# michelerenzullo/Blur_algorithms

Hardware: AMD Instinct MI355X
Metric: megapixels/sec Gaussian blur (σ=20, 4K RGB) at 1/2/4/8 GPUs; % HBM roofline (higher is better)
Workload: dtype f16 hi+lo operands (u8 pixels exact, taps and intermediate split in two binary16 halves), f32 accumulate

## Files before the change

### blur_algorithms_amd/csrc/fw_kernels.hpp

```cpp
#pragma once
#include "fx_kernels.hpp"
#include <type_traits>

#ifndef FW_TL_REGS
#define FW_TL_REGS 12
#endif

namespace blur_amd {

typedef uint32_t FwChSel;
constexpr FwChSel fw_chsel_all(int ch) { return static_cast<FwChSel>(ch) | (ch > 1 ? 0xe40u : 0u); }
inline FwChSel fw_chsel_mask(unsigned mask, int ch)
{
    FwChSel s = 0;
    int n = 0;
    for (int c = 0; c < ch; ++c)
        if (mask >> c & 1u) s |= static_cast<FwChSel>(c) << (4 + 2 * n++);
    return s | static_cast<FwChSel>(n);
}
__host__ __device__ constexpr int fw_chsel_count(FwChSel s) { return static_cast<int>(s & 7u); }
inline unsigned fw_chsel_bits(FwChSel s)
{
    unsigned m = 0;
    for (int i = 0; i < fw_chsel_count(s); ++i) m |= 1u << ((s >> (4 + 2 * i)) & 3u);
// ... 256 lines not shown
            } else {
#pragma unroll
                for (int k = 8 * hf; k < 8 * hf + 8; ++k) sv[k] = arow[k] * kFxRowUnscale;
            }
        } else if (sub == 1 || sub == 2) {
#pragma unroll
            for (int k = 4 * hf + 2 * (sub - 1); k < 4 * hf + 2 * sub; ++k) {
                typedef float f2 __attribute__((ext_vector_type(2)));
                typedef _Float16 h2 __attribute__((ext_vector_type(2)));
                const f2 vv = { sv[2 * k], sv[2 * k + 1] };
                hp[k] = __builtin_bit_cast(uint32_t, __builtin_convertvector(vv, h2));
                float r0, r1;
                mx_remainder(hp[k], vv[0], vv[1], r0, r1);
                const f2 rem = { r0, r1 };
                lp[k] = __builtin_bit_cast(uint32_t, __builtin_convertvector(rem, h2));
            }
        } else {
            fx_swap4(hp[4 * hf], hp[4 * hf + 2], hp[4 * hf + 1], hp[4 * hf + 3], lp[4 * hf], lp[4 * hf + 2], lp[4 * hf + 1], lp[4 * hf + 3]);
        }
    };
    const uint32_t sel1 = (lane & 1) ? 0x03070105u : 0x06020400u, sel2 = (lane & 2) ? 0x03020706u : 0x05040100u;
    auto emit_piece = [&](int gq) __attribute__((always_inline)) {
        float fv[4];
#pragma unroll
        for (int k = 0; k < 4; ++k) {
            const int reg = 4 * gq + k;
            fv[k] = __builtin_fmaf(tfin[reg], kMxUnscale, (reg & 1) ? cneg : cpos);
        }
        const uint32_t b0 = static_cast<uint32_t>(static_cast<int>(fv[0])) & 0xffu, b1 = static_cast<uint32_t>(static_cast<int>(fv[1])) & 0xffu;
        const uint32_t b2 = static_cast<uint32_t>(static_cast<int>(fv[2])) & 0xffu, b3 = static_cast<uint32_t>(static_cast<int>(fv[3]));
        const uint32_t pk = b0 | (b1 << 8) | (b2 << 16) | (b3 << 24);
        rr[gq] = CH == 1 ? fx_quad_transpose(pk, sel1, sel2) : pk;
    };
    auto colpass = [&](int qs, int hb, int ri, auto beside) __attribute__((always_inline)) {
        mx_half8 v1[2], v2[2];
#pragma unroll
        for (int b = 0; b < 2; ++b) {
            const u4 w1 = { hl[hb][0][4 * b], hl[hb][0][4 * b + 1], hl[hb][0][4 * b + 2], hl[hb][0][4 * b + 3] };
            const u4 w2 = { hl[hb][1][4 * b], hl[hb][1][4 * b + 1], hl[hb][1][4 * b + 2], hl[hb][1][4 * b + 3] };
            v1[b] = __builtin_bit_cast(mx_half8, w1);
            v2[b] = __builtin_bit_cast(mx_half8, w2);
        }
        auto dof = [](int it) { return it == 0 ? NKB - 1 : (it >= NKB - 2 ? it - (NKB - 2) : it + 1); };
        mx_half8 tq[3];
        tq[0] = tlo(dof(0));
        if (NKB > 1) tq[1] = tlo(dof(1));
#pragma unroll
        for (int it = 0; it < CS; ++it) {
            if (it < NKB) {
                const int d = dof(it);
                const int b = d & 1, a2 = d >> 1, slot = (qs - a2 + 2 * NT) % NT;
                if (it + 2 < NKB) tq[(it + 2) % 3] = tlo(dof(it + 2));
                if (ri < 0 || a2 <= ri) {
                    mx_float16 t = d == 0 ? zero : acc[slot];
                    t = __builtin_amdgcn_mfma_f32_32x32x16_f16(th[d], v1[b], t, 0, 0, 0);
                    t = __builtin_amdgcn_mfma_f32_32x32x16_f16(tq[it % 3], v1[b], t, 0, 0, 0);
                    t = __builtin_amdgcn_mfma_f32_32x32x16_f16(th[d], v2[b], t, 0, 0, 0);
                    asm volatile("" : "+a"(t));
                    if (it == 0) tfin = t; else acc[slot] = t;
                }
            }
            beside(it);
            __builtin_amdgcn_sched_barrier(0);
        }
    };
    const __amdgpu_buffer_rsrc_t rout = __builtin_amdgcn_make_buffer_rsrc(out, 0, static_cast<uint32_t>(g.rows - 1) * pt.dst_pitch + static_cast<uint32_t>(g.cols) * CH, kMxRsrcWord3);
    const int xcol = x0 + 32 * wave + m;
    const uint32_t lane_out = CH == 3 ? static_cast<uint32_t>(4 * h) * pt.dst_pitch + static_cast<uint32_t>(xcol) * CH + static_cast<uint32_t>(c) : 0u;
    uint32_t rowstep_ = pt.dst_pitch;
    asm volatile("" : "+s"(rowstep_));
    const uint32_t rowstep = rowstep_;
    const int xq = x0 + 32 * wave + 4 * (m >> 2), q = m & 3;
    const bool ragged = (g.cols & 3) != 0;
    const int qn = xq >= g.cols ? 0 : min(4, g.cols - xq);
    auto store_group = [&](int tile, bool valid, int gq) __attribute__((always_inline)) {
        const uint32_t v = rr[gq];
        if constexpr (CH == 1) {
            const int row = 32 * tile + 8 * gq + 4 * h + q;
            const bool rok = valid && row < g.rows;
            const uint32_t o = static_cast<uint32_t>(row) * rowstep + static_cast<uint32_t>(xq);
            __builtin_amdgcn_raw_buffer_store_b32(v, rout, rok && qn == 4 ? o : 0xfffffff0u, 0, 0);
            if (ragged) {
#pragma unroll
                for (int k = 0; k < 3; ++k)
                    __builtin_amdgcn_raw_buffer_store_b8(static_cast<uint8_t>(v >> (8 * k)), rout, rok && qn < 4 && k < qn ? o + k : 0xfffffff0u, 0, 0);
            }
        } else {
            int row0 = 32 * tile + 8 * gq + 4 * h;
            if constexpr (CH == 4) asm volatile("" : "+v"(row0));
            const uint32_t base = CH == 3 ? lane_out + static_cast<uint32_t>(32 * tile + 8 * gq) * rowstep
                                          : static_cast<uint32_t>(row0) * rowstep + static_cast<uint32_t>(xcol) * CH + static_cast<uint32_t>(c);
#pragma unroll
            for (int k = 0; k < 4; ++k) {
                const bool ok = valid && xcol < g.cols && row0 + k < g.rows;
                __builtin_amdgcn_raw_buffer_store_b8(static_cast<uint8_t>(v >> (8 * k)), rout, ok ? base + k * rowstep : 0xfffffff0u, 0, 0);
            }
        }
    };

    issue_window(s0);
#pragma unroll
    for (int k = 0; k < PER; ++k) commit_item(0, k);
    commit_q(0);
    issue_window(s0 + 1);
#pragma unroll
    for (int k = 0; k < PER; ++k) commit_item(1, k);
    commit_q(1);
    __syncthreads();
    rowpass(0, [](int) {});
#pragma unroll
    for (int p = 0; p < 8; ++p) split_piece(0, 0, p);
    __syncthreads();

    auto step = [&](int s, int qs, int ri) __attribute__((always_inline)) {
        const int par = (s - s0) & 1;
        const int ptile = s - 1 - NT;
        const bool pvalid = ptile >= tile0 && s > s0;
        issue_window(s + 2);
        rowpass(par ^ 1, [&](int kb) __attribute__((always_inline)) {
            if (kb < 4) store_group(ptile, pvalid, kb);
        });
        colpass(qs, 0, ri, [&](int it) __attribute__((always_inline)) {
            if (it < 8) split_piece(par ^ 1, 1, it);
            if (it >= 1 && it <= 4) emit_piece(it - 1);
            if (it >= 5) {
#pragma unroll
                for (int i = 0; i < IPS; ++i) commit_item(par, IPS * (it - 5) + i);
            }
            if (it == CS - 1) commit_q(par);
        });
#pragma unroll
        for (int k = 0; k < 8; ++k) { hl[0][0][k] = hl[1][0][k]; hl[0][1][k] = hl[1][1][k]; }
        __syncthreads();
    };
#pragma unroll
    for (int j = 0; j < NT; ++j) step(s0 + j, j, j);
    for (int sb = s0 + NT; sb < s1; sb += NT) {
#pragma unroll
        for (int qs = 0; qs < NT; ++qs) {
            const int s = sb + qs;
            if (s >= s1) break;
            step(s, qs, -1);
        }
    }
    {
        const int ltile = s1 - 1 - NT;
#pragma unroll
        for (int gq = 0; gq < 4; ++gq) store_group(ltile, ltile >= tile0, gq);
    }
}

template <int NKB, int CH> hipError_t fw_launch(hipStream_t st, const uint8_t* src, uint8_t* dst, const void* frags, FxGeom g, int num_cus, const FwQuirk<CH>* qk,
                                               const uint8_t* strips, FwChSel chsel, FwPitch pt)
{
    using C = FwCfg<NKB>;
    const int nact = fw_chsel_count(chsel);
    if (nact < 1 || nact > CH) return hipErrorInvalidValue;
    for (int i = 0; i < nact; ++i)
        if (static_cast<int>((chsel >> (4 + 2 * i)) & 3u) >= CH) return hipErrorInvalidValue;
    const FxLaunch l = fx_plan_launch(g, nact, C::NT, num_cus);
    if (l.ntasks == 0) return hipSuccess;
    static std::atomic<unsigned long long> attr_done{ 0 };
    const hipError_t e = fx_set_lds(attr_done, C::LDS, fw_blur_u8<NKB, true, CH>, fw_blur_u8<NKB, false, CH>);
    if (e != hipSuccess) return e;
    if (qk)
        hipLaunchKernelGGL((fw_blur_u8<NKB, true, CH>), l.grid, dim3(256), C::LDS, st, src, dst, static_cast<const mx_half8*>(frags), g, l.chunks, l.tps,
                           l.nseg, static_cast<int>(l.ntasks), *qk, strips, chsel, pt);
    else
        hipLaunchKernelGGL((fw_blur_u8<NKB, false, CH>), l.grid, dim3(256), C::LDS, st, src, dst, static_cast<const mx_half8*>(frags), g, l.chunks, l.tps,
                           l.nseg, static_cast<int>(l.ntasks), FwQuirk<CH>{}, strips, chsel, pt);
    return hipGetLastError();
}

template <int NKB> hipError_t fw_launch_u8c3(hipStream_t st, const uint8_t* src, uint8_t* dst, const void* frags, FxGeom g, int num_cus, const FxQuirk* qk,
                                             const uint8_t* strips, float* vdump, unsigned long long* stamps)
{
// ... 170 lines not shown
```

### blur_algorithms_amd/csrc/fx_kernels.hpp

```cpp
#pragma once
#include "mx_kernels.hpp"
#include <atomic>

#if !defined(FX_NO_SGB) && !defined(FX_SGB)
#define FX_SGB 1
#endif
#ifndef FX_SGB_A
#define FX_SGB_A 5
#endif
#ifndef FX_SGB_B
#define FX_SGB_B 6
#endif

namespace blur_amd {

struct FxGeom {
    int rows, cols, pad;
    int nframes;
    int aligned;
    int ntiles;
    int nright;
    int nxcd;
};

// ... 23 lines not shown
constexpr float kFxRowUnscale = 1024.f;

__host__ __device__ constexpr uint32_t fx_sel1(int B, int da, int db) { return (B >> 2) == db ? static_cast<uint32_t>(B & 3) : static_cast<uint32_t>(4 + (B & 3)); }

template <int NKB> struct FxRaw { uint32_t d[FxCfg<NKB>::PER][3]; };

__device__ __forceinline__ void fx_swap4(uint32_t& a0, uint32_t& b0, uint32_t& a1, uint32_t& b1, uint32_t& a2, uint32_t& b2, uint32_t& a3, uint32_t& b3)
{
    asm("s_nop 1\n\tv_permlane32_swap_b32 %0, %1\n\tv_permlane32_swap_b32 %2, %3\n\tv_permlane32_swap_b32 %4, %5\n\tv_permlane32_swap_b32 %6, %7"
        : "+v"(a0), "+v"(b0), "+v"(a1), "+v"(b1), "+v"(a2), "+v"(b2), "+v"(a3), "+v"(b3));
}

template <int CTRL> __device__ __forceinline__ uint32_t fx_dpp(uint32_t x)
{
    return static_cast<uint32_t>(__builtin_amdgcn_update_dpp(0, static_cast<int>(x), CTRL, 0xf, 0xf, true));
}

#ifdef FX_ABL_M16
typedef float fx_f4 __attribute__((ext_vector_type(4)));
struct fx_tile { fx_f4 q[4]; };
#define FX_EL(t, i) ((t).q[(i) >> 2][(i) & 3])
#define FX_PIN(t) asm volatile("" : "+a"((t).q[0]), "+a"((t).q[1]), "+a"((t).q[2]), "+a"((t).q[3]))
__device__ __forceinline__ void fx_mma(mx_half8 a, mx_half8 b, fx_tile& t, int pair)
{
    t.q[2 * pair] = __builtin_amdgcn_mfma_f32_16x16x32_f16(a, b, t.q[2 * pair], 0, 0, 0);
    t.q[2 * pair + 1] = __builtin_amdgcn_mfma_f32_16x16x32_f16(a, b, t.q[2 * pair + 1], 0, 0, 0);
}
#else
typedef mx_float16 fx_tile;
#define FX_EL(t, i) ((t)[i])
#define FX_PIN(t) asm volatile("" : "+a"(t))
__device__ __forceinline__ void fx_mma(mx_half8 a, mx_half8 b, fx_tile& t, int) { t = __builtin_amdgcn_mfma_f32_32x32x16_f16(a, b, t, 0, 0, 0); }
#endif

__device__ __forceinline__ uint32_t fx_quad_transpose(uint32_t p, uint32_t sel1, uint32_t sel2)
{
    const uint32_t t = fx_dpp<0xb1>(p);
    const uint32_t q = __builtin_amdgcn_perm(t, p, sel1);
    const uint32_t u = fx_dpp<0x4e>(q);
    return __builtin_amdgcn_perm(u, q, sel2);
}

struct FxQuirk {
    const int* srow_part;
    const int* cpart;
    const long long* zpart;
    const float* taps;
    int nbatches, nbands;
    int cpitch;
    float dr, dc;
};

template <int NCH>
__device__ __forceinline__ void fx_quirk_cols_tile(unsigned char* scratch, float* qc, const FxQuirk& q, int f, int x0, int c0, int cols, int pad, int tid)
{
    const int win = kFxChunk + 2 * pad, nval = NCH * win, ntap = 2 * pad + 1;
    double* cc = reinterpret_cast<double*>(scratch);
    double* tp = cc + nval;
    double* zs = tp + ntap;
    int* S = reinterpret_cast<int*>(zs + 4 + ((nval + ntap) & 1));
    const size_t bstride = static_cast<size_t>(q.cpitch);
    const int wlo = x0 - pad, whi = min(x0 + kFxChunk, cols) + pad;
    int xlo = max(wlo, 0), xhi = min(whi, cols);
    if (wlo < 0) xhi = max(xhi, min(cols, 1 - wlo));
    if (whi > cols) xlo = min(xlo, max(0, 2 * cols - 1 - whi));
    {
// ... 236 lines not shown
    };
    float sv[16];
    auto split_piece = [&](int buf, int c, int piece, int sprod = 0) __attribute__((always_inline)) {
        const int hf = piece / 4, sub = piece % 4;
        uint32_t (&hp)[8] = hl[0];
        uint32_t (&lp)[8] = hl[1];
#ifdef FX_ABL_NOSPLIT
        if (sub == 0) {
#pragma unroll
            for (int k = 0; k < 4; ++k) { hp[4 * hf + k] = __builtin_bit_cast(uint32_t, FX_EL(arow, 8 * hf + k)); lp[4 * hf + k] = __builtin_bit_cast(uint32_t, FX_EL(arow, 8 * hf + 4 + k)); }
        }
        return;
#endif
        if (sub == 0) {
            if (QUIRK) {
                const float* qs4 = reinterpret_cast<const float*>(fx_lds + C::QOFF) + buf * 512 + (m & 1) * 256 + c * 32 + 4 * h;
#pragma unroll
                for (int k = 0; k < 2; ++k) {
                    const float4 t4 = *reinterpret_cast<const float4*>(qs4 + 8 * (2 * hf + k));
                    sv[8 * hf + 4 * k] = __builtin_fmaf(FX_EL(arow, 8 * hf + 4 * k), kFxRowUnscale, t4.x);
                    sv[8 * hf + 4 * k + 1] = __builtin_fmaf(FX_EL(arow, 8 * hf + 4 * k + 1), kFxRowUnscale, t4.y);
                    sv[8 * hf + 4 * k + 2] = __builtin_fmaf(FX_EL(arow, 8 * hf + 4 * k + 2), kFxRowUnscale, t4.z);
                    sv[8 * hf + 4 * k + 3] = __builtin_fmaf(FX_EL(arow, 8 * hf + 4 * k + 3), kFxRowUnscale, t4.w);
                }
            } else {
#pragma unroll
                for (int k = 0; k < 8; ++k) sv[8 * hf + k] = FX_EL(arow, 8 * hf + k) * kFxRowUnscale;
            }
            if (DUMPV) {
                const int x = x0 + 32 * wave + m;
#pragma unroll
                for (int k = 0; k < 8; ++k) {
                    const int reg = 8 * hf + k, r = 32 * sprod + (reg & 3) + 8 * (reg >> 2) + 4 * h - PADA;
                    if (r >= 0 && r < g.rows && x < g.cols) vdump[((static_cast<size_t>(f) * 3 + c) * g.rows + r) * g.cols + x] = sv[8 * hf + k];
                }
            }
        } else if (sub == 1 || sub == 2) {
#pragma unroll
            for (int k = 2 * (sub - 1); k < 2 * sub; ++k) {
                typedef float f2 __attribute__((ext_vector_type(2)));
                typedef _Float16 h2 __attribute__((ext_vector_type(2)));
                const f2 vv = { sv[8 * hf + 2 * k], sv[8 * hf + 2 * k + 1] };
                hp[4 * hf + k] = __builtin_bit_cast(uint32_t, __builtin_convertvector(vv, h2));
                float r0, r1;
                mx_remainder(hp[4 * hf + k], vv[0], vv[1], r0, r1);
                const f2 rem = { r0, r1 };
                lp[4 * hf + k] = __builtin_bit_cast(uint32_t, __builtin_convertvector(rem, h2));
            }
        } else {
#ifndef FX_ABL_NOSWAP
            fx_swap4(hp[4 * hf], hp[4 * hf + 2], hp[4 * hf + 1], hp[4 * hf + 3], lp[4 * hf], lp[4 * hf + 2], lp[4 * hf + 1], lp[4 * hf + 3]);
#endif
        }
    };
    fx_tile tfin = zero;
    auto emit_piece = [&](int c, int gq) __attribute__((always_inline)) {
#ifdef FX_ABL_NOEMIT
        rr[c][gq] = __builtin_bit_cast(uint32_t, FX_EL(tfin, 5 * gq));
        return;
#endif
        float fv[4];
#pragma unroll
        for (int k = 0; k < 4; ++k) {
            const int reg = 4 * gq + k;
            fv[k] = __builtin_fmaf(FX_EL(tfin, reg), kMxUnscale, (reg & 1) ? cneg[c] : cpos[c]);
        }
        uint32_t pk = static_cast<uint32_t>(static_cast<int>(fv[0]));
        asm("v_cvt_i32_f32_sdwa %0, %1 dst_sel:BYTE_1 dst_unused:UNUSED_PRESERVE src0_sel:DWORD" : "+v"(pk) : "v"(fv[1]));
        asm("v_cvt_i32_f32_sdwa %0, %1 dst_sel:BYTE_2 dst_unused:UNUSED_PRESERVE src0_sel:DWORD" : "+v"(pk) : "v"(fv[2]));
        asm("v_cvt_i32_f32_sdwa %0, %1 dst_sel:BYTE_3 dst_unused:UNUSED_PRESERVE src0_sel:DWORD" : "+v"(pk) : "v"(fv[3]));
        rr[c][gq] = fx_quad_transpose(pk, sel1, sel2);
    };
    auto colpass = [&](int c, int qs, int ri, auto beside) __attribute__((always_inline)) {
        typedef uint32_t u4 __attribute__((ext_vector_type(4)));
        mx_half8 v1[2], v2[2];
#pragma unroll
        for (int b = 0; b < 2; ++b) {
            const u4 w1 = { hl[0][4 * b], hl[0][4 * b + 1], hl[0][4 * b + 2], hl[0][4 * b + 3] };
            const u4 w2 = { hl[1][4 * b], hl[1][4 * b + 1], hl[1][4 * b + 2], hl[1][4 * b + 3] };
            v1[b] = __builtin_bit_cast(mx_half8, w1);
            v2[b] = __builtin_bit_cast(mx_half8, w2);
        }
#pragma unroll
        for (int it = 0; it < NKB; ++it) {
            const int d = it == 0 ? NKB - 1 : (it >= NKB - 2 ? it - (NKB - 2) : it + 1);
            const int b = d & 1, a2 = d >> 1, slot = (qs - a2 + 2 * NT) % NT;
            if (ri < 0 || a2 <= ri) {
                fx_tile t = d == 0 ? zero : acc[c][slot];
                fx_mma(th[d], v1[b], t, 0);
                fx_mma(tl[d], v1[b], t, 1);
                fx_mma(th[d], v2[b], t, 0);
                FX_PIN(t);
                if (it == 0) tfin = t; else acc[c][slot] = t;
            }
            beside(it);
#ifdef FX_SGB
            __builtin_amdgcn_sched_group_barrier(0x008, 1, 0);
            __builtin_amdgcn_sched_group_barrier(0x002, FX_SGB_B, 0);
            __builtin_amdgcn_sched_group_barrier(0x008, 1, 0);
            __builtin_amdgcn_sched_group_barrier(0x002, FX_SGB_B, 0);
            __builtin_amdgcn_sched_group_barrier(0x008, 1, 0);
            __builtin_amdgcn_sched_group_barrier(0x002, FX_SGB_B, 0);
#endif
#ifndef FX_NOSB
            __builtin_amdgcn_sched_barrier(0);
#endif
        }
    };
    const __amdgpu_buffer_rsrc_t rout = __builtin_amdgcn_make_buffer_rsrc(out, 0, static_cast<uint32_t>(g.rows) * g.cols * 3u, kMxRsrcWord3);
    const uint32_t lane_out = (static_cast<uint32_t>(4 * h + q) * g.cols + static_cast<uint32_t>(xpix)) * 3u;
    auto store_group = [&](int tile, bool valid, int gq) __attribute__((always_inline)) {
        {
            const uint32_t r0 = rr[0][gq], r1 = rr[1][gq], r2 = rr[2][gq];
            const uint32_t X = __builtin_amdgcn_perm(r1, r0, 0x05010400u);
            const uint32_t Y = __builtin_amdgcn_perm(r1, r0, 0x07030602u);
            const uint32_t w0 = __builtin_amdgcn_perm(r2, X, 0x02040100u);
            const uint32_t Z = __builtin_amdgcn_perm(r2, X, 0x0c0c0503u);
            const uint32_t w1 = __builtin_amdgcn_perm(Y, Z, 0x05040100u);
            const uint32_t w2 = __builtin_amdgcn_perm(r2, Y, 0x07030206u);
            typedef uint32_t u3 __attribute__((ext_vector_type(3)));
// ... 25 lines not shown
    if (QUIRK) {
        static_assert(C::BUF >= 8 * (3 * C::WIN + 2 * PADA + 1 + 6) + 4 * (3 * C::WIN + 4), "fx_quirk_cols_tile's scratch fits window buffer 0");
        float* qc = reinterpret_cast<float*>(fx_lds + C::BUF);
        fx_quirk_cols_tile<3>(fx_lds, qc, qk, f, x0, 0, g.cols, g.pad, tid);
#pragma unroll
        for (int c = 0; c < 3; ++c) {
            const float v = qc[3 * (32 * wave + m) + c];
            cpos[c] = 0.5f + v;
            cneg[c] = 0.5f - v;
        }
        __syncthreads();
    } else {
#pragma unroll
        for (int c = 0; c < 3; ++c) cpos[c] = cneg[c] = 0.5f;
    }
#pragma unroll
    for (int j = 0; j < 3; ++j) commit_chunk(0, j);
    issue_chunk(s0 + 1, 0);
    commit_chunk(1, 0);
    issue_chunk(s0 + 1, 1);
    issue_chunk(s0 + 1, 2);
    issue_chunk(s0 + 2, 0);
    __syncthreads();
    rowpass(0, 0, [](int) {});
    split_piece(0, 0, 0, s0);
    split_piece(0, 0, 4, s0);

#ifdef FX_STAMPS
    unsigned long long st_acc[6] = { 0, 0, 0, 0, 0, 0 }, st_prev = __builtin_amdgcn_s_memtime(), st_begin = st_prev;
#define FX_STAMP(i) { const unsigned long long t_ = __builtin_amdgcn_s_memtime(); st_acc[i] += t_ - st_prev; st_prev = t_; }
#else
#define FX_STAMP(i)
#endif
    auto step = [&](int s, int qs, int ri) __attribute__((always_inline)) {
        {
            const int cur = (s - s0) & 1;
#pragma unroll
            for (int c = 0; c < 3; ++c) {
#ifndef FX_ABL_NOBARRIER
                if (c == 2) __syncthreads();
#endif
#ifndef FX_NOSB
                __builtin_amdgcn_sched_barrier(0);
#endif
                {
                    const int jc = c == 2 ? 0 : c + 1, cbuf = c == 2 ? cur : cur ^ 1, snext = c == 2 ? s + 3 : s + 2;
                    const bool tvalid = s - 1 - NT >= tile0 && s > s0;
                    constexpr int NI = NKB >= 11 ? 1 : (NKB >= 6 ? 2 : (NKB >= 4 ? 3 : 5));
                    auto beside = [&](int kb) __attribute__((always_inline)) {
                        if (NKB >= 11) {
                            if (kb == 0) split_piece(cur, c, 1);
                            if (kb == 1) split_piece(cur, c, 2);
                            if (kb == 2) { split_piece(cur, c, 3); split_piece(cur, c, 5); }
                            if (kb == 3) split_piece(cur, c, 6);
                            if (kb == 4) split_piece(cur, c, 7);
                            if (c == 0 && kb >= 5 && kb <= 8) store_group(s - 1 - NT, tvalid, kb - 5);
#ifdef FX_NO_BALANCE
                            if (kb >= 2) commit_item(cbuf, 3 * jc + (kb - 2) / 3, (kb - 2) % 3);
                            if (kb == NKB - 1) { if (jc == 0) commit_q(cbuf); issue_chunk(snext, jc); }
#else
                            (void)jc; (void)cbuf; (void)snext;
#endif
                        } else {
                            if (kb == 0) { split_piece(cur, c, 1); split_piece(cur, c, 2); split_piece(cur, c, 3); split_piece(cur, c, 5); split_piece(cur, c, 6); split_piece(cur, c, 7); }
#pragma unroll
                            for (int i = NI * kb; i < NI * kb + NI && i < 9; ++i) commit_item(cbuf, 3 * jc + i / 3, i % 3);
                            if (kb == NKB - 1) { if (jc == 0) commit_q(cbuf); issue_chunk(snext, jc); }
                            if (c == 0 && kb == NKB - 1) store_tile(s - 1 - NT, tvalid);
                        }
                    };
                    if (c == 2) rowpass(cur ^ 1, 0, beside); else rowpass(cur, c + 1, beside);
                }
#ifndef FX_NOSB
                __builtin_amdgcn_sched_barrier(0);
#endif
                FX_STAMP(2 * c)
                {
                    const int nbuf = c == 2 ? cur ^ 1 : cur, nc = c == 2 ? 0 : c + 1;
                    auto beside = [&](int it) __attribute__((always_inline)) {
                        if (NKB >= 11) {
                            if (it == 1) split_piece(nbuf, nc, 0, c == 2 ? s + 1 : s);
                            if (it == 2) split_piece(nbuf, nc, 4, c == 2 ? s + 1 : s);
                            if (it >= 3 && it <= 6) emit_piece(c, it - 3);
#ifndef FX_NO_BALANCE
                            {
                                const int jc = c == 2 ? 0 : c + 1, cbuf = c == 2 ? cur : cur ^ 1, snext = c == 2 ? s + 3 : s + 2;
                                const int sl = it == 0 ? 0 : it - 6;
                                if (it == 0 || it >= 7) {
                                    commit_item(cbuf, 3 * jc + (2 * sl) / 3, (2 * sl) % 3);
                                    if (sl < 4) commit_item(cbuf, 3 * jc + (2 * sl + 1) / 3, (2 * sl + 1) % 3);
                                }
                                if (it == NKB - 1) { if (jc == 0) commit_q(cbuf); issue_chunk(snext, jc); }
                            }
#endif
                        } else {
                            if (it == (NKB >= 5 ? 1 : 0)) { split_piece(nbuf, nc, 0, c == 2 ? s + 1 : s); split_piece(nbuf, nc, 4, c == 2 ? s + 1 : s); }
                            if (it == (NKB >= 5 ? NKB - 3 : 0)) {
#pragma unroll
                                for (int gq = 0; gq < 4; ++gq) emit_piece(c, gq);
                            }
                        }
                    };
                    colpass(c, qs, ri, beside);
                }
#ifndef FX_NOSB
                __builtin_amdgcn_sched_barrier(0);
#endif
                FX_STAMP(2 * c + 1)
            }
        }
    };
#ifndef FX_NO_PEEL
#pragma unroll
    for (int j = 0; j < NT; ++j) step(s0 + j, j, j);
    for (int sb = s0 + NT; sb < s1; sb += NT) {
#else
    for (int sb = s0; sb < s1; sb += NT) {
#endif
#pragma unroll
        for (int qs = 0; qs < NT; ++qs) {
            const int s = sb + qs;
            if (s >= s1) break;
            step(s, qs, -1);
        }
    }
    store_tile(s1 - 1 - NT, s1 - 1 - NT >= tile0);
#ifdef FX_STAMPS
    if (!QUIRK && !DUMPV && vdump && blockIdx.x == 0 && tid == 0) {
        unsigned long long* o = reinterpret_cast<unsigned long long*>(vdump);
        for (int i = 0; i < 6; ++i) o[i] = st_acc[i];
        o[6] = __builtin_amdgcn_s_memtime() - st_begin;
        o[7] = static_cast<unsigned long long>(s1 - s0);
    }
#endif
}

#ifdef BLUR_FX_QUIRK_KERNELS
inline int fx_right_strips(int cols, int pada)
{
    const int chunks = (cols + kFxChunk - 1) / kFxChunk;
    int n = 0;
    for (int xc = chunks - 1; xc >= fx_left_strips(pada) && kFxChunk * xc + kFxChunk + pada > cols; --xc) ++n;
    return n;
}

__device__ __forceinline__ void fx_edge_strips_body(const uint8_t* __restrict__ src, uint8_t* __restrict__ strips, int rows, int cols, int pada, int chunks, int nright,
                                                    int bx, int sidx, int f, int narrow, uint32_t spitch, size_t sframe)
{
    const int win = kFxChunk + 2 * pada, gpr = win / 4;
    const int nleft = fx_left_strips(pada);
    const int xc = sidx < nleft ? sidx : chunks - nright + sidx - nleft, x0 = kFxChunk * xc;
    int glo = 0, gn = gpr;
    if (narrow) {
        int lo, hi;
        fx_strip_range(xc, cols, pada, (gpr + 7) / 8, &lo, &hi);
        glo = 8 * lo;
        gn = min(8 * hi, gpr) - glo;
    }
// ... 56 lines not shown
    int br = kFxSumRows;
#ifndef FX_BAND_WGS
#define FX_BAND_WGS 4
#endif
    while (br < 128 && nbatches * ((rows + 2 * br - 1) / (2 * br)) * nframes >= static_cast<long long>(FX_BAND_WGS) * num_cus) br *= 2;
    return br;
}

template <int G>
__device__ __forceinline__ void fx_altsums_body(const uint8_t* __restrict__ src, int* __restrict__ srow_part, int* __restrict__ cpart, long long* __restrict__ zpart,
                                                int rows, int cols, int pad, int nbands, int nbatches, int band, int batch, int f, int (*sred)[3][64], int band_rows,
                                                uint32_t spitch, size_t sframe)
{
    const int tid = threadIdx.x;
    const uint8_t* img = src + static_cast<size_t>(f) * sframe;
    const __amdgpu_buffer_rsrc_t rimg = __builtin_amdgcn_make_buffer_rsrc(const_cast<uint8_t*>(img), 0, static_cast<uint32_t>(rows - 1) * spitch + static_cast<uint32_t>(cols) * 3u, kMxRsrcWord3);
    const int groups = (cols + 3) / 4, r0 = band * band_rows, r1 = min(r0 + band_rows, rows);
    const int flip = (pad & 1) ? -1 : 1;
    const int over = (4 - (cols & 3)) & 3;
    int gi[G], wq[G][4];
    bool act[G], plain[G], last[G];
    uint32_t col0[G];
#pragma unroll
    for (int j = 0; j < G; ++j) {
        gi[j] = (batch * G + j) * 256 + tid;
        act[j] = gi[j] < groups;
        last[j] = over != 0 && gi[j] == groups - 1;
        const int x = 4 * gi[j] - (last[j] ? over : 0);
        plain[j] = !last[j] && x > pad && x + 3 < cols - 1 - pad;
#pragma unroll
        for (int q = 0; q < 4; ++q) wq[j][q] = (act[j] && !(last[j] && q < over)) ? mx_alt_weight(x + q, cols, pad) : 0;
        col0[j] = act[j] ? 3u * static_cast<uint32_t>(x) : 0u;
    }
    int o[G][12];
#pragma unroll
    for (int j = 0; j < G; ++j)
#pragma unroll
        for (int k = 0; k < 12; ++k) o[j][k] = 0;
    long long zacc = 0;
    typedef uint32_t u3 __attribute__((ext_vector_type(3)));
    for (int rs = r0; rs < r1; rs += kFxSumRows) {
        const int re = min(rs + kFxSumRows, r1);
        for (int i = tid; i < kFxSumRows * 3 * 64; i += 256) (&sred[0][0][0])[i] = 0;
        __syncthreads();
        uint32_t accp[G][6], accn[G][6];
#pragma unroll
        for (int j = 0; j < G; ++j)
#pragma unroll
            for (int k = 0; k < 6; ++k) accp[j][k] = accn[j][k] = 0;
#ifndef FX_PRE_RB
#define FX_PRE_RB 8
#endif
        constexpr int RB = G == 1 ? FX_PRE_RB : (G == 2 ? 4 : 2);
        for (int rb = rs; rb < re; rb += RB) {
            u3 d[RB][G];
#pragma unroll
            for (int i = 0; i < RB; ++i) {
                const int r = min(rb + i, re - 1);
#pragma unroll
                for (int j = 0; j < G; ++j) d[i][j] = __builtin_amdgcn_raw_buffer_load_b96(rimg, col0[j] + static_cast<uint32_t>(r) * spitch, 0, 0);
            }
#pragma unroll
            for (int i = 0; i < RB; ++i) {
                const int r = rb + i;
                if (r < re) {
                    const int wy = mx_alt_weight(r, rows, pad);
                    const uint32_t aw = static_cast<uint32_t>(wy < 0 ? -wy : wy);
                    int s[3] = { 0, 0, 0 };
#pragma unroll
                    for (int j = 0; j < G; ++j) {
                        const u3 dd = d[i][j];
                        if (plain[j]) {
                            const int e0 = static_cast<int>(dd[0] ^ 0x80808080u), e1 = static_cast<int>(dd[1] ^ 0x80808080u), e2 = static_cast<int>(dd[2] ^ 0x80808080u);
                            int t0 = __builtin_amdgcn_sdot4(e0, static_cast<int>(0xff000001u), 0, false);
                            t0 = __builtin_amdgcn_sdot4(e1, 0x00010000, t0, false);
                            t0 = __builtin_amdgcn_sdot4(e2, 0x0000ff00, t0, false);
                            int t1 = __builtin_amdgcn_sdot4(e0, 0x00000100, 0, false);
                            t1 = __builtin_amdgcn_sdot4(e1, 0x010000ff, t1, false);
                            t1 = __builtin_amdgcn_sdot4(e2, 0x00ff0000, t1, false);
                            int t2 = __builtin_amdgcn_sdot4(e0, 0x00010000, 0, false);
                            t2 = __builtin_amdgcn_sdot4(e1, 0x0000ff00, t2, false);
                            t2 = __builtin_amdgcn_sdot4(e2, static_cast<int>(0xff000001u), t2, false);
                            s[0] += flip * t0; s[1] += flip * t1; s[2] += flip * t2;
                        } else {
#pragma unroll
                            for (int q = 0; q < 4; ++q)
#pragma unroll
                                for (int c = 0; c < 3; ++c) {
                                    const int byte = 3 * q + c;
                                    s[c] += wq[j][q] * static_cast<int>((dd[byte >> 2] >> (8 * (byte & 3))) & 0xffu);
                                }
                        }
#pragma unroll
                        for (int k = 0; k < 3; ++k) {
                            uint32_t lo = __builtin_amdgcn_perm(0u, dd[k], 0x0c020c00u), hi = __builtin_amdgcn_perm(0u, dd[k], 0x0c030c01u);
                            if (aw != 1) { lo *= aw; hi *= aw; }
                            if (wy > 0) { accp[j][2 * k] += lo; accp[j][2 * k + 1] += hi; }
                            else { accn[j][2 * k] += lo; accn[j][2 * k + 1] += hi; }
                        }
                    }
#pragma unroll
                    for (int c = 0; c < 3; ++c) atomicAdd(&sred[r - rs][c][tid & 63], s[c]);
                }
            }
        }
#pragma unroll
        for (int j = 0; j < G; ++j)
#pragma unroll
            for (int k = 0; k < 3; ++k) {
                o[j][4 * k] += static_cast<int>(accp[j][2 * k] & 0xffffu) - static_cast<int>(accn[j][2 * k] & 0xffffu);
                o[j][4 * k + 2] += static_cast<int>(accp[j][2 * k] >> 16) - static_cast<int>(accn[j][2 * k] >> 16);
                o[j][4 * k + 1] += static_cast<int>(accp[j][2 * k + 1] & 0xffffu) - static_cast<int>(accn[j][2 * k + 1] & 0xffffu);
                o[j][4 * k + 3] += static_cast<int>(accp[j][2 * k + 1] >> 16) - static_cast<int>(accn[j][2 * k + 1] >> 16);
            }
        __syncthreads();
        if (tid < (re - rs) * 3) {
            const int* p64 = &sred[0][0][0] + 64 * tid;
            int v = 0;
#pragma unroll 8
            for (int k = 0; k < 64; ++k) v += p64[(k + tid) & 63];
            srow_part[((static_cast<size_t>(f) * nbatches + batch) * rows + rs) * 3 + tid] = v;
            zacc += static_cast<long long>(mx_alt_weight(rs + tid / 3, rows, pad)) * v;
        }
        __syncthreads();
    }
    if (over != 0) {
#pragma unroll
        for (int j = 0; j < G; ++j)
#pragma unroll
            for (int k = 0; k < 9; ++k) {
                const int v3 = o[j][k + 3], v6 = k + 6 < 12 ? o[j][k + 6] : 0, v9 = k + 9 < 12 ? o[j][k + 9] : 0;
                o[j][k] = last[j] ? (over == 1 ? v3 : (over == 2 ? v6 : v9)) : o[j][k];
            }
    }
#pragma unroll
    for (int j = 0; j < G; ++j)
        if (act[j]) {
            int4* dstp = reinterpret_cast<int4*>(cpart + (static_cast<size_t>(f) * nbands + band) * (12 * static_cast<size_t>(groups)) + 12 * gi[j]);
            dstp[0] = make_int4(o[j][0], o[j][1], o[j][2], o[j][3]);
            dstp[1] = make_int4(o[j][4], o[j][5], o[j][6], o[j][7]);
            dstp[2] = make_int4(o[j][8], o[j][9], o[j][10], o[j][11]);
        }
    long long* zs = reinterpret_cast<long long*>(&sred[0][0][0]);
    if (tid < 96) zs[tid] = zacc;
    __syncthreads();
    if (tid < 3) {
        long long z = 0;
        for (int k = 0; k < kFxSumRows; ++k) z += zs[3 * k + tid];
        zpart[((static_cast<size_t>(f) * nbands + band) * nbatches + batch) * 3 + tid] = z;
    }
}

template <int G>
__global__ __launch_bounds__(256) void fx_prepass(const uint8_t* __restrict__ src, int* __restrict__ srow_part, int* __restrict__ cpart, long long* __restrict__ zpart,
                                                  uint8_t* __restrict__ strips, int rows, int cols, int pad, int pada, int nbands, int nbatches, int n_alt, int chunks,
                                                  int nright, int strip_blocks, int band_rows, int narrow, uint32_t spitch, size_t sframe)
{
    __shared__ int sred[kFxSumRows][3][64];
    int b = blockIdx.x;
    if (b < n_alt) {
        const int band = b % nbands, batch = (b / nbands) % nbatches, f = b / (nbands * nbatches);
        fx_altsums_body<G>(src, srow_part, cpart, zpart, rows, cols, pad, nbands, nbatches, band, batch, f, sred, band_rows, spitch, sframe);
    } else {
        b -= n_alt;
        const int nstrips = fx_left_strips(pada) + nright, bx = b % strip_blocks, sidx = (b / strip_blocks) % nstrips, f = b / (strip_blocks * nstrips);
        fx_edge_strips_body(src, strips, rows, cols, pada, chunks, nright, bx, sidx, f, narrow, spitch, sframe);
    }
}
#endif

struct FxLaunch {
    int chunks = 0, nseg = 1, tps = 0;
    long long ntasks = 0;
    dim3 grid;
};
inline FxLaunch fx_plan_launch(FxGeom& g, int nch, int nt, int num_cus)
{
    FxLaunch l;
    l.chunks = (g.cols + kFxChunk - 1) / kFxChunk;
    const long long nstripes = static_cast<long long>(l.chunks) * g.nframes * nch;
    if (nstripes <= 0) return l;
    l.tps = g.ntiles;
    long long best = -1;
    for (int n = 1; n <= g.ntiles; ++n) {
        const int t = (g.ntiles + n - 1) / n, ns = (g.ntiles + t - 1) / t;
        const long long rounds = (nstripes * ns + num_cus - 1) / num_cus, span = rounds * (t + nt);
        if (best < 0 || span < best) { best = span; l.nseg = ns; l.tps = t; }
// ... 61 lines not shown
```

Baseline: 192,500.

## Peel final NT steps to skip dead MFMAs and prefetches in run-out

Splits the main tile loop so the last NT steps run as a peeled run-out phase. In that phase, column-pass MFMAs for accumulator slots whose output rows lie past the strip end are skipped. Global prefetch issues and LDS commits for tiles that will never be consumed are also dropped. To keep the slot indexing consistent, the accumulator tiles are rotated in AGPRs at run-out entry by the runtime phase, which adds accvgpr moves and nops plus extra unrolled code size.

```diff
diff --git a/blur_algorithms_amd/csrc/fw_kernels.hpp b/blur_algorithms_amd/csrc/fw_kernels.hpp
--- a/blur_algorithms_amd/csrc/fw_kernels.hpp
+++ b/blur_algorithms_amd/csrc/fw_kernels.hpp
@@ -312,7 +312,7 @@
         const uint32_t pk = b0 | (b1 << 8) | (b2 << 16) | (b3 << 24);
         rr[gq] = CH == 1 ? fx_quad_transpose(pk, sel1, sel2) : pk;
     };
-    auto colpass = [&](int qs, int hb, int ri, auto beside) __attribute__((always_inline)) {
+    auto colpass = [&](int qs, int hb, int ri, int ro, auto beside) __attribute__((always_inline)) {
         mx_half8 v1[2], v2[2];
 #pragma unroll
         for (int b = 0; b < 2; ++b) {
@@ -331,7 +331,7 @@
                 const int d = dof(it);
                 const int b = d & 1, a2 = d >> 1, slot = (qs - a2 + 2 * NT) % NT;
                 if (it + 2 < NKB) tq[(it + 2) % 3] = tlo(dof(it + 2));
-                if (ri < 0 || a2 <= ri) {
+                if ((ri < 0 || a2 <= ri) && a2 > ro) {
                     mx_float16 t = d == 0 ? zero : acc[slot];
                     t = __builtin_amdgcn_mfma_f32_32x32x16_f16(th[d], v1[b], t, 0, 0, 0);
                     t = __builtin_amdgcn_mfma_f32_32x32x16_f16(tq[it % 3], v1[b], t, 0, 0, 0);
@@ -392,36 +392,46 @@
     for (int p = 0; p < 8; ++p) split_piece(0, 0, p);
     __syncthreads();
 
-    auto step = [&](int s, int qs, int ri) __attribute__((always_inline)) {
+    auto step = [&](int s, int qs, int ri, int ro) __attribute__((always_inline)) {
         const int par = (s - s0) & 1;
         const int ptile = s - 1 - NT;
         const bool pvalid = ptile >= tile0 && s > s0;
-        issue_window(s + 2);
+        const bool stage = ro < 0 || ro + 2 <= NT - 1;
+        if (stage) issue_window(s + 2);
         rowpass(par ^ 1, [&](int kb) __attribute__((always_inline)) {
             if (kb < 4) store_group(ptile, pvalid, kb);
         });
-        colpass(qs, 0, ri, [&](int it) __attribute__((always_inline)) {
+        colpass(qs, 0, ri, ro, [&](int it) __attribute__((always_inline)) {
             if (it < 8) split_piece(par ^ 1, 1, it);
             if (it >= 1 && it <= 4) emit_piece(it - 1);
             if (it >= 5) {
 #pragma unroll
-                for (int i = 0; i < IPS; ++i) commit_item(par, IPS * (it - 5) + i);
-            }
-            if (it == CS - 1) commit_q(par);
+                for (int i = 0; i < IPS; ++i)
+                    if (stage) commit_item(par, IPS * (it - 5) + i);
+            }
+            if (it == CS - 1 && stage) commit_q(par);
         });
 #pragma unroll
         for (int k = 0; k < 8; ++k) { hl[0][0][k] = hl[1][0][k]; hl[0][1][k] = hl[1][1][k]; }
         __syncthreads();
     };
 #pragma unroll
-    for (int j = 0; j < NT; ++j) step(s0 + j, j, j);
-    for (int sb = s0 + NT; sb < s1; sb += NT) {
+    for (int j = 0; j < NT; ++j) step(s0 + j, j, j, -1);
+    const bool runout = tile1 - tile0 >= NT;
+    const int sm = runout ? s1 - NT : s1;
+    for (int sb = s0 + NT; sb < sm; sb += NT) {
 #pragma unroll
         for (int qs = 0; qs < NT; ++qs) {
             const int s = sb + qs;
-            if (s >= s1) break;
-            step(s, qs, -1);
-        }
+            if (s >= sm) break;
+            step(s, qs, -1, -1);
+        }
+    }
+    if (runout) {
+        const int ph = (sm - s0) % NT;
+        fx_rebase_tiles<1, NT>(&acc, ph);
+#pragma unroll
+        for (int j = 0; j < NT; ++j) step(sm + j, j, -1, j);
     }
     {
         const int ltile = s1 - 1 - NT;
diff --git a/blur_algorithms_amd/csrc/fx_kernels.hpp b/blur_algorithms_amd/csrc/fx_kernels.hpp
--- a/blur_algorithms_amd/csrc/fx_kernels.hpp
+++ b/blur_algorithms_amd/csrc/fx_kernels.hpp
@@ -79,6 +79,35 @@
 #define FX_PIN(t) asm volatile("" : "+a"(t))
 __device__ __forceinline__ void fx_mma(mx_half8 a, mx_half8 b, fx_tile& t, int) { t = __builtin_amdgcn_mfma_f32_32x32x16_f16(a, b, t, 0, 0, 0); }
 #endif
+
+__host__ __device__ constexpr int fx_gcd(int a, int b) { return b == 0 ? a : fx_gcd(b, a % b); }
+template <int NT, int P> __device__ __forceinline__ void fx_rotate_tiles(fx_tile (&a)[NT])
+{
+    constexpr int NCYC = fx_gcd(NT, P), LEN = NT / NCYC;
+#pragma unroll
+    for (int c0 = 0; c0 < NCYC; ++c0) {
+#pragma unroll
+        for (int i = 0; i < 16; ++i) {
+            float tmp;
+            asm volatile("v_accvgpr_read_b32 %0, %1" : "=v"(tmp) : "a"(FX_EL(a[c0], i)));
+#pragma unroll
+            for (int j = 0; j < LEN - 1; ++j)
+                asm volatile("v_accvgpr_mov_b32 %0, %1" : "+a"(FX_EL(a[(c0 + j * P) % NT], i)) : "a"(FX_EL(a[(c0 + (j + 1) * P) % NT], i)));
+            asm volatile("v_accvgpr_write_b32 %0, %1" : "+a"(FX_EL(a[(c0 + (LEN - 1) * P) % NT], i)) : "v"(tmp));
+        }
+    }
+}
+template <int NC, int NT, int P = 1> __device__ __forceinline__ void fx_rebase_tiles(fx_tile (*a)[NT], int ph)
+{
+    if constexpr (P == 1) asm volatile("s_nop 7\n\ts_nop 7\n\ts_nop 3");
+    if constexpr (P < NT) {
+        if (ph & P) {
+#pragma unroll
+            for (int c = 0; c < NC; ++c) fx_rotate_tiles<NT, P>(a[c]);
+        }
+        fx_rebase_tiles<NC, NT, 2 * P>(a, ph);
+    }
+}
 
 __device__ __forceinline__ uint32_t fx_quad_transpose(uint32_t p, uint32_t sel1, uint32_t sel2)
 {
@@ -381,7 +410,7 @@
 #pragma unroll
                 for (int k = 0; k < 8; ++k) {
                     const int reg = 8 * hf + k, r = 32 * sprod + (reg & 3) + 8 * (reg >> 2) + 4 * h - PADA;
-                    if (r >= 0 && r < g.rows && x < g.cols) vdump[((static_cast<size_t>(f) * 3 + c) * g.rows + r) * g.cols + x] = sv[8 * hf + k];
+                    if (sprod < s1 && r >= 0 && r < g.rows && x < g.cols) vdump[((static_cast<size_t>(f) * 3 + c) * g.rows + r) * g.cols + x] = sv[8 * hf + k];
                 }
             }
         } else if (sub == 1 || sub == 2) {
@@ -420,7 +449,7 @@
         asm("v_cvt_i32_f32_sdwa %0, %1 dst_sel:BYTE_3 dst_unused:UNUSED_PRESERVE src0_sel:DWORD" : "+v"(pk) : "v"(fv[3]));
         rr[c][gq] = fx_quad_transpose(pk, sel1, sel2);
     };
-    auto colpass = [&](int c, int qs, int ri, auto beside) __attribute__((always_inline)) {
+    auto colpass = [&](int c, int qs, int ri, int ro, auto beside) __attribute__((always_inline)) {
         typedef uint32_t u4 __attribute__((ext_vector_type(4)));
         mx_half8 v1[2], v2[2];
 #pragma unroll
@@ -434,7 +463,7 @@
         for (int it = 0; it < NKB; ++it) {
             const int d = it == 0 ? NKB - 1 : (it >= NKB - 2 ? it - (NKB - 2) : it + 1);
             const int b = d & 1, a2 = d >> 1, slot = (qs - a2 + 2 * NT) % NT;
-            if (ri < 0 || a2 <= ri) {
+            if ((ri < 0 || a2 <= ri) && a2 > ro) {
                 fx_tile t = d == 0 ? zero : acc[c][slot];
                 fx_mma(th[d], v1[b], t, 0);
                 fx_mma(tl[d], v1[b], t, 1);
@@ -526,11 +555,12 @@
 #else
 #define FX_STAMP(i)
 #endif
-    auto step = [&](int s, int qs, int ri) __attribute__((always_inline)) {
+    auto step = [&](int s, int qs, int ri, int ro) __attribute__((always_inline)) {
         {
             const int cur = (s - s0) & 1;
 #pragma unroll
             for (int c = 0; c < 3; ++c) {
+                const bool stage_c = ro < 0 || ro + (c == 2 ? 2 : 1) <= NT - 1, stage_i = ro < 0 || ro + (c == 2 ? 3 : 2) <= NT - 1;
 #ifndef FX_ABL_NOBARRIER
                 if (c == 2) __syncthreads();
 #endif
@@ -539,6 +569,7 @@
 #endif
                 {
                     const int jc = c == 2 ? 0 : c + 1, cbuf = c == 2 ? cur : cur ^ 1, snext = c == 2 ? s + 3 : s + 2;
+                    (void)stage_c; (void)stage_i;
                     const bool tvalid = s - 1 - NT >= tile0 && s > s0;
                     constexpr int NI = NKB >= 11 ? 1 : (NKB >= 6 ? 2 : (NKB >= 4 ? 3 : 5));
                     auto beside = [&](int kb) __attribute__((always_inline)) {
@@ -550,16 +581,17 @@
                             if (kb == 4) split_piece(cur, c, 7);
                             if (c == 0 && kb >= 5 && kb <= 8) store_group(s - 1 - NT, tvalid, kb - 5);
 #ifdef FX_NO_BALANCE
-                            if (kb >= 2) commit_item(cbuf, 3 * jc + (kb - 2) / 3, (kb - 2) % 3);
-                            if (kb == NKB - 1) { if (jc == 0) commit_q(cbuf); issue_chunk(snext, jc); }
+                            if (kb >= 2 && stage_c) commit_item(cbuf, 3 * jc + (kb - 2) / 3, (kb - 2) % 3);
+                            if (kb == NKB - 1) { if (jc == 0 && stage_c) commit_q(cbuf); if (stage_i) issue_chunk(snext, jc); }
 #else
                             (void)jc; (void)cbuf; (void)snext;
 #endif
                         } else {
                             if (kb == 0) { split_piece(cur, c, 1); split_piece(cur, c, 2); split_piece(cur, c, 3); split_piece(cur, c, 5); split_piece(cur, c, 6); split_piece(cur, c, 7); }
 #pragma unroll
-                            for (int i = NI * kb; i < NI * kb + NI && i < 9; ++i) commit_item(cbuf, 3 * jc + i / 3, i % 3);
-                            if (kb == NKB - 1) { if (jc == 0) commit_q(cbuf); issue_chunk(snext, jc); }
+                            for (int i = NI * kb; i < NI * kb + NI && i < 9; ++i)
+                                if (stage_c) commit_item(cbuf, 3 * jc + i / 3, i % 3);
+                            if (kb == NKB - 1) { if (jc == 0 && stage_c) commit_q(cbuf); if (stage_i) issue_chunk(snext, jc); }
                             if (c == 0 && kb == NKB - 1) store_tile(s - 1 - NT, tvalid);
                         }
                     };
@@ -580,11 +612,11 @@
                             {
                                 const int jc = c == 2 ? 0 : c + 1, cbuf = c == 2 ? cur : cur ^ 1, snext = c == 2 ? s + 3 : s + 2;
                                 const int sl = it == 0 ? 0 : it - 6;
-                                if (it == 0 || it >= 7) {
+                                if ((it == 0 || it >= 7) && stage_c) {
                                     commit_item(cbuf, 3 * jc + (2 * sl) / 3, (2 * sl) % 3);
                                     if (sl < 4) commit_item(cbuf, 3 * jc + (2 * sl + 1) / 3, (2 * sl + 1) % 3);
                                 }
-                                if (it == NKB - 1) { if (jc == 0) commit_q(cbuf); issue_chunk(snext, jc); }
+                                if (it == NKB - 1) { if (jc == 0 && stage_c) commit_q(cbuf); if (stage_i) issue_chunk(snext, jc); }
                             }
 #endif
                         } else {
@@ -595,7 +627,7 @@
                             }
                         }
                     };
-                    colpass(c, qs, ri, beside);
+                    colpass(c, qs, ri, ro, beside);
                 }
 #ifndef FX_NOSB
                 __builtin_amdgcn_sched_barrier(0);
@@ -606,18 +638,37 @@
     };
 #ifndef FX_NO_PEEL
 #pragma unroll
-    for (int j = 0; j < NT; ++j) step(s0 + j, j, j);
-    for (int sb = s0 + NT; sb < s1; sb += NT) {
+    for (int j = 0; j < NT; ++j) step(s0 + j, j, j, -1);
+#ifndef FX_NO_RUNOUT
+    const bool runout = tile1 - tile0 >= NT;
+#else
+    const bool runout = false;
+#endif
+    const int sm = runout ? s1 - NT : s1;
+    for (int sb = s0 + NT; sb < sm; sb += NT) {
+#pragma unroll
+        for (int qs = 0; qs < NT; ++qs) {
+            const int s = sb + qs;
+            if (s >= sm) break;
+            step(s, qs, -1, -1);
+        }
+    }
+    if (runout) {
+        const int ph = (sm - s0) % NT;
+        fx_rebase_tiles<3, NT>(acc, ph);
+#pragma unroll
+        for (int j = 0; j < NT; ++j) step(sm + j, j, -1, j);
+    }
 #else
     for (int sb = s0; sb < s1; sb += NT) {
-#endif
 #pragma unroll
         for (int qs = 0; qs < NT; ++qs) {
             const int s = sb + qs;
             if (s >= s1) break;
-            step(s, qs, -1);
-        }
-    }
+            step(s, qs, -1, -1);
+        }
+    }
+#endif
     store_tile(s1 - 1 - NT, s1 - 1 - NT >= tile0);
 #ifdef FX_STAMPS
     if (!QUIRK && !DUMPV && vdump && blockIdx.x == 0 && tid == 0) {
```

Measured after the change: 191,000, median of 2. About the same (-0.8%).

## Software-pipeline row loads and add wave-uniform fast path in alt-sum prepass

Applied to the files above, without the earlier changes.

Restructures the prepass alternating-sum body so that row loads are issued one tile ahead, using an out-of-bounds offset for rows past the band. When every column in a wavefront is interior and the rows are interior, a fast path skips the per-row weight and sign branches. The flip sign is folded into the dot-product weight constants, and accumulators are split by row parity instead of by weight sign. The shared reduction is reworked to use int4 reads with a DPP pair-add, clearing the buffer as it goes, and launch bounds gain an occupancy hint. In exchange, register pressure rises from the prefetch buffers and the parity-based sign mapping assumes |weight| is 1 on the fast path.

```diff
diff --git a/blur_algorithms_amd/csrc/fx_kernels.hpp b/blur_algorithms_amd/csrc/fx_kernels.hpp
--- a/blur_algorithms_amd/csrc/fx_kernels.hpp
+++ b/blur_algorithms_amd/csrc/fx_kernels.hpp
@@ -740,6 +740,12 @@
         for (int q = 0; q < 4; ++q) wq[j][q] = (act[j] && !(last[j] && q < over)) ? mx_alt_weight(x + q, cols, pad) : 0;
         col0[j] = act[j] ? 3u * static_cast<uint32_t>(x) : 0u;
     }
+    bool allplain = true;
+#pragma unroll
+    for (int j = 0; j < G; ++j) allplain = allplain && plain[j];
+    const bool wave_plain = __builtin_amdgcn_ballot_w64(!allplain) == 0;
+    const int wA = flip > 0 ? static_cast<int>(0xff000001u) : 0x010000ff, wB = flip > 0 ? 0x00010000 : 0x00ff0000, wC = flip > 0 ? 0x0000ff00 : 0x00000100;
+    const int wD = flip > 0 ? 0x00000100 : 0x0000ff00, wE = flip > 0 ? 0x010000ff : static_cast<int>(0xff000001u), wF = flip > 0 ? 0x00ff0000 : 0x00010000;
     int o[G][12];
 #pragma unroll
     for (int j = 0; j < G; ++j)
@@ -747,88 +753,136 @@
         for (int k = 0; k < 12; ++k) o[j][k] = 0;
     long long zacc = 0;
     typedef uint32_t u3 __attribute__((ext_vector_type(3)));
+    constexpr int RB = G == 4 ? 2 : 4;
+    constexpr uint32_t kOob = 0xfff00000u;
+    u3 d[RB][G];
+    auto load_row = [&](int i, int r) {
+        const uint32_t roff = r < r1 ? static_cast<uint32_t>(r) * spitch : kOob;
+#pragma unroll
+        for (int j = 0; j < G; ++j) d[i][j] = __builtin_amdgcn_raw_buffer_load_b96(rimg, col0[j] + roff, 0, 0);
+    };
+    uint32_t acc[2][G][6];
+    auto trip = [&](int rb, int rs, int re) {
+        if (wave_plain && rb > pad && rb + RB <= re && rb + RB <= rows - 1 - pad) {
+#pragma unroll
+            for (int i = 0; i < RB; ++i) {
+                int s0 = 0, s1 = 0, s2 = 0;
+#pragma unroll
+                for (int j = 0; j < G; ++j) {
+                    const u3 dd = d[i][j];
+                    const int e0 = static_cast<int>(dd[0] ^ 0x80808080u), e1 = static_cast<int>(dd[1] ^ 0x80808080u), e2 = static_cast<int>(dd[2] ^ 0x80808080u);
+                    s0 = __builtin_amdgcn_sdot4(e0, wA, s0, false);
+                    s0 = __builtin_amdgcn_sdot4(e1, wB, s0, false);
+                    s0 = __builtin_amdgcn_sdot4(e2, wC, s0, false);
+                    s1 = __builtin_amdgcn_sdot4(e0, wD, s1, false);
+                    s1 = __builtin_amdgcn_sdot4(e1, wE, s1, false);
+                    s1 = __builtin_amdgcn_sdot4(e2, wF, s1, false);
+                    s2 = __builtin_amdgcn_sdot4(e0, wB, s2, false);
+                    s2 = __builtin_amdgcn_sdot4(e1, wC, s2, false);
+                    s2 = __builtin_amdgcn_sdot4(e2, wA, s2, false);
+#pragma unroll
+                    for (int k = 0; k < 3; ++k) {
+                        acc[i & 1][j][2 * k] += __builtin_amdgcn_perm(0u, dd[k], 0x0c020c00u);
+                        acc[i & 1][j][2 * k + 1] += __builtin_amdgcn_perm(0u, dd[k], 0x0c030c01u);
+                    }
+                }
+                atomicAdd(&sred[rb - rs + i][0][tid & 63], s0);
+                atomicAdd(&sred[rb - rs + i][1][tid & 63], s1);
+                atomicAdd(&sred[rb - rs + i][2][tid & 63], s2);
+                load_row(i, rb + RB + i);
+            }
+            return;
+        }
+#pragma unroll
+        for (int i = 0; i < RB; ++i) {
+            const int r = rb + i;
+            if (r < re) {
+                const int wy = mx_alt_weight(r, rows, pad);
+                const uint32_t aw = static_cast<uint32_t>(wy < 0 ? -wy : wy);
+                int s[3] = { 0, 0, 0 };
+#pragma unroll
+                for (int j = 0; j < G; ++j) {
+                    const u3 dd = d[i][j];
+                    if (plain[j]) {
+                        const int e0 = static_cast<int>(dd[0] ^ 0x80808080u), e1 = static_cast<int>(dd[1] ^ 0x80808080u), e2 = static_cast<int>(dd[2] ^ 0x80808080u);
+                        s[0] = __builtin_amdgcn_sdot4(e0, wA, s[0], false);
+                        s[0] = __builtin_amdgcn_sdot4(e1, wB, s[0], false);
+                        s[0] = __builtin_amdgcn_sdot4(e2, wC, s[0], false);
+                        s[1] = __builtin_amdgcn_sdot4(e0, wD, s[1], false);
+                        s[1] = __builtin_amdgcn_sdot4(e1, wE, s[1], false);
+                        s[1] = __builtin_amdgcn_sdot4(e2, wF, s[1], false);
+                        s[2] = __builtin_amdgcn_sdot4(e0, wB, s[2], false);
+                        s[2] = __builtin_amdgcn_sdot4(e1, wC, s[2], false);
+                        s[2] = __builtin_amdgcn_sdot4(e2, wA, s[2], false);
+                    } else {
+#pragma unroll
+                        for (int q = 0; q < 4; ++q)
+#pragma unroll
+                            for (int c = 0; c < 3; ++c) {
+                                const int byte = 3 * q + c;
+                                s[c] += wq[j][q] * static_cast<int>((dd[byte >> 2] >> (8 * (byte & 3))) & 0xffu);
+                            }
+                    }
+#pragma unroll
+                    for (int k = 0; k < 3; ++k) {
+                        uint32_t lo = __builtin_amdgcn_perm(0u, dd[k], 0x0c020c00u), hi = __builtin_amdgcn_perm(0u, dd[k], 0x0c030c01u);
+                        if (aw != 1) { lo *= aw; hi *= aw; }
+                        acc[i & 1][j][2 * k] += lo;
+                        acc[i & 1][j][2 * k + 1] += hi;
+                    }
+                }
+#pragma unroll
+                for (int c = 0; c < 3; ++c) atomicAdd(&sred[r - rs][c][tid & 63], s[c]);
+            }
+            load_row(i, r + RB);
+        }
+    };
+#pragma unroll
+    for (int i = 0; i < RB; ++i) load_row(i, r0 + i);
+    {
+        int4* z4 = reinterpret_cast<int4*>(&sred[0][0][0]);
+        for (int i = tid; i < kFxSumRows * 3 * 64 / 4; i += 256) z4[i] = make_int4(0, 0, 0, 0);
+    }
+    __syncthreads();
     for (int rs = r0; rs < r1; rs += kFxSumRows) {
         const int re = min(rs + kFxSumRows, r1);
-        for (int i = tid; i < kFxSumRows * 3 * 64; i += 256) (&sred[0][0][0])[i] = 0;
+#pragma unroll
+        for (int h = 0; h < 2; ++h)
+#pragma unroll
+            for (int j = 0; j < G; ++j)
+#pragma unroll
+                for (int k = 0; k < 6; ++k) acc[h][j][k] = 0;
+        for (int rb = rs; rb < re; rb += RB) trip(rb, rs, re);
+        const bool podd = (pad & 1) != 0;
+#pragma unroll
+        for (int j = 0; j < G; ++j)
+#pragma unroll
+            for (int k = 0; k < 3; ++k) {
+                const uint32_t p0 = podd ? acc[1][j][2 * k] : acc[0][j][2 * k], n0 = podd ? acc[0][j][2 * k] : acc[1][j][2 * k];
+                const uint32_t p1 = podd ? acc[1][j][2 * k + 1] : acc[0][j][2 * k + 1], n1 = podd ? acc[0][j][2 * k + 1] : acc[1][j][2 * k + 1];
+                o[j][4 * k] += static_cast<int>(p0 & 0xffffu) - static_cast<int>(n0 & 0xffffu);
+                o[j][4 * k + 2] += static_cast<int>(p0 >> 16) - static_cast<int>(n0 >> 16);
+                o[j][4 * k + 1] += static_cast<int>(p1 & 0xffffu) - static_cast<int>(n1 & 0xffffu);
+                o[j][4 * k + 3] += static_cast<int>(p1 >> 16) - static_cast<int>(n1 >> 16);
+            }
         __syncthreads();
-        uint32_t accp[G][6], accn[G][6];
-#pragma unroll
-        for (int j = 0; j < G; ++j)
-#pragma unroll
-            for (int k = 0; k < 6; ++k) accp[j][k] = accn[j][k] = 0;
-#ifndef FX_PRE_RB
-#define FX_PRE_RB 8
-#endif
-        constexpr int RB = G == 1 ? FX_PRE_RB : (G == 2 ? 4 : 2);
-        for (int rb = rs; rb < re; rb += RB) {
-            u3 d[RB][G];
-#pragma unroll
-            for (int i = 0; i < RB; ++i) {
-                const int r = min(rb + i, re - 1);
-#pragma unroll
-                for (int j = 0; j < G; ++j) d[i][j] = __builtin_amdgcn_raw_buffer_load_b96(rimg, col0[j] + static_cast<uint32_t>(r) * spitch, 0, 0);
-            }
-#pragma unroll
-            for (int i = 0; i < RB; ++i) {
-                const int r = rb + i;
-                if (r < re) {
-                    const int wy = mx_alt_weight(r, rows, pad);
-                    const uint32_t aw = static_cast<uint32_t>(wy < 0 ? -wy : wy);
-                    int s[3] = { 0, 0, 0 };
-#pragma unroll
-                    for (int j = 0; j < G; ++j) {
-                        const u3 dd = d[i][j];
-                        if (plain[j]) {
-                            const int e0 = static_cast<int>(dd[0] ^ 0x80808080u), e1 = static_cast<int>(dd[1] ^ 0x80808080u), e2 = static_cast<int>(dd[2] ^ 0x80808080u);
-                            int t0 = __builtin_amdgcn_sdot4(e0, static_cast<int>(0xff000001u), 0, false);
-                            t0 = __builtin_amdgcn_sdot4(e1, 0x00010000, t0, false);
-                            t0 = __builtin_amdgcn_sdot4(e2, 0x0000ff00, t0, false);
-                            int t1 = __builtin_amdgcn_sdot4(e0, 0x00000100, 0, false);
-                            t1 = __builtin_amdgcn_sdot4(e1, 0x010000ff, t1, false);
-                            t1 = __builtin_amdgcn_sdot4(e2, 0x00ff0000, t1, false);
-                            int t2 = __builtin_amdgcn_sdot4(e0, 0x00010000, 0, false);
-                            t2 = __builtin_amdgcn_sdot4(e1, 0x0000ff00, t2, false);
-                            t2 = __builtin_amdgcn_sdot4(e2, static_cast<int>(0xff000001u), t2, false);
-                            s[0] += flip * t0; s[1] += flip * t1; s[2] += flip * t2;
-                        } else {
-#pragma unroll
-                            for (int q = 0; q < 4; ++q)
-#pragma unroll
-                                for (int c = 0; c < 3; ++c) {
-                                    const int byte = 3 * q + c;
-                                    s[c] += wq[j][q] * static_cast<int>((dd[byte >> 2] >> (8 * (byte & 3))) & 0xffu);
-                                }
-                        }
-#pragma unroll
-                        for (int k = 0; k < 3; ++k) {
-                            uint32_t lo = __builtin_amdgcn_perm(0u, dd[k], 0x0c020c00u), hi = __builtin_amdgcn_perm(0u, dd[k], 0x0c030c01u);
-                            if (aw != 1) { lo *= aw; hi *= aw; }
-                            if (wy > 0) { accp[j][2 * k] += lo; accp[j][2 * k + 1] += hi; }
-                            else { accn[j][2 * k] += lo; accn[j][2 * k + 1] += hi; }
-                        }
-                    }
-#pragma unroll
-                    for (int c = 0; c < 3; ++c) atomicAdd(&sred[r - rs][c][tid & 63], s[c]);
-                }
-            }
-        }
-#pragma unroll
-        for (int j = 0; j < G; ++j)
-#pragma unroll
-            for (int k = 0; k < 3; ++k) {
-                o[j][4 * k] += static_cast<int>(accp[j][2 * k] & 0xffffu) - static_cast<int>(accn[j][2 * k] & 0xffffu);
-                o[j][4 * k + 2] += static_cast<int>(accp[j][2 * k] >> 16) - static_cast<int>(accn[j][2 * k] >> 16);
-                o[j][4 * k + 1] += static_cast<int>(accp[j][2 * k + 1] & 0xffffu) - static_cast<int>(accn[j][2 * k + 1] & 0xffffu);
-                o[j][4 * k + 3] += static_cast<int>(accp[j][2 * k + 1] >> 16) - static_cast<int>(accn[j][2 * k + 1] >> 16);
-            }
-        __syncthreads();
-        if (tid < (re - rs) * 3) {
-            const int* p64 = &sred[0][0][0] + 64 * tid;
+        if (tid < 192) {
+            const int out = tid >> 1;
+            int4* p4 = reinterpret_cast<int4*>(&sred[0][0][0]);
+            int first = (16 * out + 8 * (tid & 1)) | (out & 7);
+            asm volatile("" : "+v"(first));
             int v = 0;
-#pragma unroll 8
-            for (int k = 0; k < 64; ++k) v += p64[(k + tid) & 63];
-            srow_part[((static_cast<size_t>(f) * nbatches + batch) * rows + rs) * 3 + tid] = v;
-            zacc += static_cast<long long>(mx_alt_weight(rs + tid / 3, rows, pad)) * v;
+#pragma unroll
+            for (int k = 0; k < 8; ++k) {
+                const int4 q4 = p4[first ^ k];
+                p4[first ^ k] = make_int4(0, 0, 0, 0);
+                v += (q4.x + q4.y) + (q4.z + q4.w);
+            }
+            v += __builtin_amdgcn_update_dpp(0, v, 0xb1, 0xf, 0xf, true);
+            if ((tid & 1) == 0 && out < (re - rs) * 3) {
+                srow_part[((static_cast<size_t>(f) * nbatches + batch) * rows + rs) * 3 + out] = v;
+                zacc += static_cast<long long>(mx_alt_weight(rs + out / 3, rows, pad)) * v;
+            }
         }
         __syncthreads();
     }
@@ -850,7 +904,7 @@
             dstp[2] = make_int4(o[j][8], o[j][9], o[j][10], o[j][11]);
         }
     long long* zs = reinterpret_cast<long long*>(&sred[0][0][0]);
-    if (tid < 96) zs[tid] = zacc;
+    if (tid < 192 && (tid & 1) == 0) zs[tid >> 1] = zacc;
     __syncthreads();
     if (tid < 3) {
         long long z = 0;
@@ -860,7 +914,7 @@
 }
 
 template <int G>
-__global__ __launch_bounds__(256) void fx_prepass(const uint8_t* __restrict__ src, int* __restrict__ srow_part, int* __restrict__ cpart, long long* __restrict__ zpart,
+__global__ __launch_bounds__(256, G <= 2 ? 3 : 2) void fx_prepass(const uint8_t* __restrict__ src, int* __restrict__ srow_part, int* __restrict__ cpart, long long* __restrict__ zpart,
                                                   uint8_t* __restrict__ strips, int rows, int cols, int pad, int pada, int nbands, int nbatches, int n_alt, int chunks,
                                                   int nright, int strip_blocks, int band_rows, int narrow, uint32_t spitch, size_t sframe)
 {
```

Result: no change. 190,300 before, 193,700 after, median of 4 (+1.8%).
